# hasindu2008/squigulator

Measured on AMD Instinct MI355X. Metric: simulated raw samples/sec, higher is better.
Workload: dtype f32+f64

## Files before the change

squigulator_amd/csrc/h_common.h:

```cpp
#pragma once

#if defined(SQG_DEV)
#define SQG_DEV_ENV(name) getenv(name)
#else
#define SQG_DEV_ENV(name) (static_cast<const char*>(nullptr))
#endif
static inline int dev_env_int(const char* v, int dflt) { return v ? atoi(v) : dflt; }

#ifndef SQG_SOURCE_HASH
#define SQG_SOURCE_HASH "unstamped"
#endif
extern "C" const char sqg_source_hash_marker[] = "SQG_SOURCE_HASH=" SQG_SOURCE_HASH ";";
#if defined(SQG_DEV)
static const char kBuildInfo[] = "source_hash=" SQG_SOURCE_HASH ";dev=1";
#else
static const char kBuildInfo[] = "source_hash=" SQG_SOURCE_HASH ";dev=0";
#endif
extern "C" const char* sqg_build_info(void) { return kBuildInfo; }

#include "h_cpus.h"

static uint32_t lcg_pow(uint32_t base, unsigned long long e) {
    uint32_t r = 1, b = base;
    while (e) { if (e & 1) r = lcg_mul(r, b); b = lcg_mul(b, b); e >>= 1; }
// ... 69 lines not shown
        int* d_slow = nullptr; size_t slow_cap = 0;
        ItemDesc* d_items = nullptr; size_t items_cap = 0;
        uint32_t* d_part = nullptr; size_t part_cap = 0;
        uint32_t* d_lbase = nullptr; size_t lbase_cap = 0;
        int* d_tile_link = nullptr; size_t tile_link_cap = 0;
        uint32_t* d_part_state = nullptr; size_t part_state_cap = 0;
        hipEvent_t cal_a = nullptr, cal_b = nullptr; bool cal_pending = false; long long cal_events = 0; int cal_tries = 0; float cal_ps = 0.f;
        uint2* cal_prev = nullptr; float cal_prev_ps = 0.f;
        unsigned long long gen = 0;
        hipEvent_t done = nullptr;
        hipEvent_t sampled = nullptr;
    } slot[2];
    struct CountSet {
        uint16_t* d_dwell = nullptr; size_t dwell_cap = 0;
        uint32_t* d_tile_so = nullptr; size_t tile_cap = 0;
        unsigned long long* d_seglen = nullptr; size_t seglen_cap = 0;
        size_t seglen_dirty = 0;
        unsigned long long gen = 0;
    } cset[3];
    int num_cu = 256;
    std::deque<sqg_batch*> staged_q;
    hipStream_t fix_stream = nullptr;
    unsigned long long* d_scan_part = nullptr; size_t scan_part_cap = 0;
    uint32_t* d_link_rows = nullptr; size_t link_rows_cap = 0;
    uint32_t* d_pcnt[2] = {nullptr, nullptr}; size_t pcnt_cap[2] = {0, 0};
    uint32_t* d_slice = nullptr; size_t slice_cap = 0;
    uint32_t* d_phist = nullptr; size_t phist_cap = 0;
    double row_bound = 0;
    bool range_mode = false;
    uint32_t* d_xcounts = nullptr; size_t xcounts_cap = 0;
// ... 269 lines not shown
```

squigulator_amd/csrc/h_context.h:

```cpp
#pragma once

extern "C" const char* sqg_strerror(int code) {
    switch (code) {
    case SQG_OK: return "ok";
    case SQG_EINVAL: return "invalid argument or unsupported configuration";
    case SQG_ENOMEM: return "out of memory";
    case SQG_EDEVICE: return "HIP runtime error";
    case SQG_ESEQUENCE: return "batches must be run in staging order";
    case SQG_ENODEVICE: return "no usable HIP device";
    case SQG_EOVERFLOW: return "read too long (>= UINT32_MAX samples) or dwell > 65535";
    case SQG_EIO: return "file I/O error";
    default: return "unknown error";
    }
}

extern "C" const char* sqg_last_error(const sqg_ctx_t* ctx) { return ctx ? ctx->err.c_str() : ""; }

extern "C" int sqg_device_count(void) {
    int n = 0;
    if (hipGetDeviceCount(&n) != hipSuccess) return SQG_ENODEVICE;
    return n;
}

extern "C" int32_t sqg_worker_of(int32_t i, int32_t n_rec, int32_t T) {
    if (T <= 1 || n_rec <= 0) return 0;
    const int32_t step = (n_rec + T - 1) / T;
    return i / step;
}

extern "C" void sqg_destroy(sqg_ctx_t* ctx) {
    if (!ctx) return;
    if (ctx->b5_reader_drain) ctx->b5_reader_drain(ctx->b5_reader, true);
    (void)hipSetDevice(ctx->cfg.device);
    if (ctx->b5_stream) { (void)hipStreamSynchronize(ctx->b5_stream); (void)hipStreamDestroy(ctx->b5_stream); ctx->b5_stream = nullptr; }
    if (ctx->stream) (void)hipStreamSynchronize(ctx->stream);
    if (ctx->fix_stream) (void)hipStreamSynchronize(ctx->fix_stream);
    delete ctx->draw_ahead; ctx->draw_ahead = nullptr;
    (void)hipFree(ctx->d_pcnt[0]); (void)hipFree(ctx->d_pcnt[1]); (void)hipFree(ctx->d_slice); (void)hipFree(ctx->d_phist);
    (void)hipFree(ctx->d_rows); (void)hipFree(ctx->d_link_rows); (void)hipFree(ctx->d_scan_part); (void)hipFree(ctx->d_xcounts); (void)hipFree(ctx->d_model); (void)hipFree(ctx->d_samp_scratch); (void)hipFree(ctx->d_pow); (void)hipFree(ctx->d_err); (void)hipFree(ctx->d_mid_done); if (ctx->h_samp) (void)hipHostFree(ctx->h_samp);
    for (auto& Q : ctx->cset) { (void)hipFree(Q.d_dwell); (void)hipFree(Q.d_tile_so); (void)hipFree(Q.d_seglen); }
    for (auto& S : ctx->slot) {
        (void)hipFree(S.d_sig); (void)hipFree(S.d_sigoff);
        (void)hipFree(S.d_fix); (void)hipFree(S.d_fix_count); (void)hipFree(S.d_fix_sh); (void)hipFree(S.d_fix_sh_count);
        (void)hipFree(S.d_evrec); (void)hipFree(S.d_slow);
        (void)hipFree(S.d_items); (void)hipFree(S.d_part_state); (void)hipFree(S.d_part); (void)hipFree(S.d_lbase); (void)hipFree(S.d_tile_link);
        (void)hipFree(S.cal_prev);
        if (S.cal_a) (void)hipEventDestroy(S.cal_a);
        if (S.cal_b) (void)hipEventDestroy(S.cal_b);
        if (S.done) (void)hipEventDestroy(S.done);
        if (S.sampled) (void)hipEventDestroy(S.sampled);
    }
    (void)hipFree(ctx->d_svb); (void)hipFree(ctx->d_svb_size); (void)hipFree(ctx->d_svb_off);
    (void)hipFree(ctx->d_b5meta); (void)hipFree(ctx->d_b5out); (void)hipFree(ctx->d_b5tab); (void)hipFree(ctx->d_b5size); for (auto* q : ctx->h_b5out) if (q) (void)hipHostFree(q); if (ctx->h_b5meta) (void)hipHostFree(ctx->h_b5meta);
    (void)hipFree(ctx->d_chunk_off); (void)hipFree(ctx->d_chunk_const); (void)hipFree(ctx->d_chunk_read); (void)hipFree(ctx->d_chunk_ev); (void)hipFree(ctx->d_chunk_wide); (void)hipFree(ctx->d_chunk_ghist); (void)hipFree(ctx->d_target_start);
    (void)hipFree(ctx->d_genome); (void)hipFree(ctx->d_contig_off); (void)hipFree(ctx->d_cum); (void)hipFree(ctx->d_nprefix);
// ... 178 lines not shown
```

squigulator_amd/csrc/h_results.h:

```cpp
#pragma once

static bool slot_is_mine(const sqg_ctx* c, const sqg_batch* b) { return c->slot[b->slot].gen == b->slot_gen; }
static bool cset_is_mine(const sqg_ctx* c, const sqg_batch* b) { return c->cset[b->cset].gen == b->cset_gen; }

extern "C" int sqg_batch_wait(sqg_ctx_t* c, sqg_batch_t* b, sqg_result_t* res) {
    if (!c || !b || !b->ran) return SQG_EINVAL;
    HIPCHK(c, hipSetDevice(c->cfg.device));
    HIPCHK(c, hipEventSynchronize(b->ev[4]));
    sqg_ctx::Slot& S = c->slot[b->slot];
    if (!b->waited) {
        b->n_samples = b->h_sigoff[b->n];
        for (int i = 0; i <= b->n; i++) b->sig_off[(size_t)i] = b->h_sigoff[i];
        unsigned int e = 0;
        const unsigned int* const hres = reinterpret_cast<const unsigned int*>(b->h_sigoff + (b->h_n - SQG_HRES_LL));
        if (b->fixup_launched) e = hres[0];
        else HIPCHK(c, hipMemcpy(&e, b->d_err, sizeof e, hipMemcpyDeviceToHost));
        b->waited = true;
        if (e) {
            c->err = "device reported: " + std::string((e & 1) ? "dwell>65535 " : "") + ((e & 2) ? "read>=UINT32_MAX samples " : "") + ((e & 4) ? "internal length mismatch " : "") + ((e & 8) ? "FP64 fix-up list overflow " : "") + ((e & 32) ? "one k-mer stream asked for >= 2^32 samples by one batch " : "") +
                     ((e & 64) ? "LDS atomics were not served in lane order (the batch's sample of the stream hand-out; create the context with SQG_ORDER_FREE) " : "") +
                     ((e & 0x80000000u) ? "the batch's last kernel left no report" : "");
            b->wait_rc = (e & (12 | 64 | 0x80000000u)) ? SQG_EDEVICE : SQG_EOVERFLOW;
            return b->wait_rc;
        }
// ... 47 lines not shown

extern "C" int sqg_fetch_dwell(sqg_ctx_t* c, sqg_batch_t* b, int32_t* dst) {
    if (!c || !b || !b->ran || !dst) return SQG_EINVAL;
    if (b->run_idx + 2 < c->runs || !slot_is_mine(c, b) || !cset_is_mine(c, b)) return SQG_ESEQUENCE;
    HIPCHK(c, hipSetDevice(c->cfg.device));
    HIPCHK(c, hipEventSynchronize(b->ev[4]));
    if (!c->use_dwell_stream) {
        for (long long i = 0; i < b->n_events; i++) dst[i] = (int)c->cfg.profile.dwell_mean;
        return SQG_OK;
    }
    std::vector<uint16_t> tmp((size_t)b->n_events);
    if (b->n_events) HIPCHK(c, hipMemcpy(tmp.data(), c->cset[b->cset].d_dwell, tmp.size() * sizeof(uint16_t), hipMemcpyDeviceToHost));
    for (size_t i = 0; i < tmp.size(); i++) dst[i] = tmp[i];
    return SQG_OK;
}

extern "C" int sqg_get_timing(sqg_ctx_t* c, sqg_timing_t* t) {
    if (!c || !t) return SQG_EINVAL;
    *t = c->timing;
    return SQG_OK;
}

extern "C" int sqg_set_phase_timing(sqg_ctx_t* c, int every) {
    if (!c || every < 0) return SQG_EINVAL;
    c->phase_timing_every = every;
    return SQG_OK;
}

extern "C" int sqg_set_stage_threads(sqg_ctx_t* c, int n) {
    if (!c || n < 0 || n > 64) return SQG_EINVAL;
// ... 194 lines not shown
```

squigulator_amd/csrc/h_run.h:

```cpp
#pragma once

static void count_params(sqg_ctx* c, const sqg_batch* b, sqg_ctx::CountSet& Q, const int n_part, uint32_t* d_pcnt, SigParams& P) {
    const sqg_profile_t& p = c->cfg.profile;
    P.reads = b->d_reads; P.chain_off = b->d_chain_off; P.chain_reads = b->d_chain_reads; P.chain_order = b->d_chain_order; P.bases = b->d_bases;
    P.dwell = c->use_dwell_stream ? Q.d_dwell : nullptr; P.dwell_out = Q.d_dwell; P.seglen_out = Q.d_seglen; P.seglen = Q.d_seglen; P.tile_so = Q.d_tile_so;
    P.dmean = p.dwell_mean; P.dstd = p.dwell_std; P.pw = c->d_pow; P.err = b->d_err; P.delta_x = c->delta_x;
    P.k = c->k; P.num_kmer = c->num_kmer; P.const_sps = (int)p.dwell_mean;
    P.dwell_unbounded = c->dwell_hi > 65535.0 ? 1 : 0;
    P.dwell_pack = c->dwell_hi < 1024.0 ? 1 : 0;
    P.pieces = b->d_pieces; P.piece_total = b->d_piece_total;
    P.pcnt = d_pcnt; P.n_part = n_part; P.n_links = b->n_chains;
}

struct RunStep { const char* name; std::function<int()> go; };
typedef std::vector<RunStep> RunPlan;

struct Run {
    sqg_ctx* c; sqg_batch* b; int phase; const uint32_t* before; const uint32_t* after;
    sqg_ctx::Slot* S; sqg_ctx::Slot* other; sqg_ctx::CountSet* Q;
    int n = 0, n_part = 0, dw = 0;
    bool certified = false, direct = false, fold = false, untimed = false, wave_links = false;
    size_t n_pairs = 0, n_rows = 0;
    unsigned scan_wgs = 0, pgrid = 0;
    uint32_t *d_pcnt = nullptr, *slice_lo = nullptr, *slice_hi = nullptr, *pfirst = nullptr, *pstart = nullptr, *ptotal = nullptr;
// ... 103 lines not shown
    P.part = S.d_part; P.part_state = b->part ? S.d_part_state : nullptr;
    P.poff = b->one ? b->d_link_slot : R.d_pcnt ? R.d_pcnt + (size_t)b->n_chains * n_part : nullptr;
    P.link_q = b->d_link_q;
    P.one = b->one ? 1 : 0;
    count_params(c, b, Q, n_part, R.d_pcnt, P);
    P.pstart = R.pstart;
    P.sig_off = S.d_sigoff; P.model = c->d_model; P.rows = c->d_rows;
    P.seed_base = canon((long long)c->cfg.seed + (long long)c->wlo * ((long long)c->num_kmer + 10)); P.seed_step = canon((long long)c->num_kmer + 10);
    P.dig = p.digitisation; P.range = p.range; P.kd = p.digitisation / p.range;
    P.thr_all = c->thr_all;
    P.meth = (c->cfg.flags & SQG_METH) ? 1 : 0; P.num_kmer_pad = n_part * PART_SUB;
    P.meth_top = 1; for (int i = 1; i < c->k; i++) P.meth_top *= 5u;
    P.use_streams = c->use_kmer_streams ? 1 : 0;
    P.rna = (c->cfg.flags & SQG_RNA) ? 1 : 0;
    P.evrec = S.d_evrec;
    if (b->part && b->pieces && !b->one) { P.evrec32 = reinterpret_cast<uint32_t*>(S.d_evrec); P.lbase = S.d_lbase; P.tile_link = S.d_tile_link; }
    P.tile_read = b->d_tile_read; P.stile_read = b->d_stile_read;
    const bool rna_prefix = (c->cfg.flags & SQG_RNA) && (c->cfg.flags & SQG_PREFIX);
    P.shift_len = rna_prefix ? (int)strlen(kAdaptorRna) * (int)p.dwell_mean : 0;
    {
        const double v = 30 * p.digitisation / p.range;
        int32_t t = (v > -2147483649.0 && v < 2147483648.0) ? (int32_t)v : (int32_t)0x80000000u;
        P.shift = (int)(int16_t)(uint16_t)((uint32_t)t & 0xffffu);
    }
    P.slow_count = S.d_fix_count + 1; P.items = S.d_items; P.lean_epl = c->lean_epl;
    P.slow_tiles = (R.certified && c->use_kmer_streams) ? S.d_slow : nullptr;
    R.fold = phase == 0 && n > 0 && b->n_chains > 0 && b->part && !b->one && b->pieces && R.certified && c->use_kmer_streams;
    memset(&R.SA, 0, sizeof R.SA);
    if (n > 0 && phase != 1) {
        ScanArgs& SA = R.SA;
        SA.seglen = Q.d_seglen; SA.n_reads = n; SA.sig_off = S.d_sigoff; SA.host_off = b->h_sigoff_dev; SA.err = b->d_err; SA.counters = S.d_fix_count;
// ... 24 lines not shown
    const dim3 g((unsigned)((b->n_chains + PEV_WAVES - 1) / PEV_WAVES)), t(64 * PEV_WAVES);
    if (!count) hipLaunchKernelGGL((k_part_events<0, PEV_SCATTER>), dim3((unsigned)((b->n_chains + PEV_WAVES_SCATTER - 1) / PEV_WAVES_SCATTER)), dim3(64 * PEV_WAVES_SCATTER), 0, c->stream, P, b->n_chains, (uint32_t)b->n_events);
    else if (b->one) {
        if (dwm == 0) hipLaunchKernelGGL((k_part_events<0, PEV_ONE>), g, t, 0, c->stream, P, b->n_chains, (uint32_t)b->n_events);
        else if (dwm == 1) hipLaunchKernelGGL((k_part_events<1, PEV_ONE>), g, t, 0, c->stream, P, b->n_chains, (uint32_t)b->n_events);
        else hipLaunchKernelGGL((k_part_events<2, PEV_ONE>), g, t, 0, c->stream, P, b->n_chains, (uint32_t)b->n_events);
    }
    else if (dwm == 0) hipLaunchKernelGGL((k_part_events<0, PEV_COUNT>), g, t, 0, c->stream, P, b->n_chains, (uint32_t)b->n_events);
    else if (dwm == 1) hipLaunchKernelGGL((k_part_events<1, PEV_COUNT>), g, t, 0, c->stream, P, b->n_chains, (uint32_t)b->n_events);
    else hipLaunchKernelGGL((k_part_events<2, PEV_COUNT>), g, t, 0, c->stream, P, b->n_chains, (uint32_t)b->n_events);
}
#define PLACE_TRIES 3
static int place_calibrate(Run& R) {
    sqg_ctx* c = R.c; sqg_batch* b = R.b; sqg_ctx::Slot& S = *R.S;
    static const bool off = SQG_DEV_ENV("SQG_NO_PLACE") != nullptr;
    if (off || c->cal_runs_left <= 0 || !R.wave_links || !R.P.evrec32 || b->n_events < (1ll << 24)) return SQG_OK;
    if (!S.cal_a) { HIPCHK(c, hipEventCreate(&S.cal_a)); HIPCHK(c, hipEventCreate(&S.cal_b)); }
    if (S.cal_pending) {
        float ms = 0.f;
        HIPCHK(c, hipEventSynchronize(S.cal_b));
        HIPCHK(c, hipEventElapsedTime(&ms, S.cal_a, S.cal_b));
        S.cal_pending = false;
        float ps = ms * 1.0e9f / (float)S.cal_events;
        const char* what = "";
        if (S.cal_prev) {
            if (ps > S.cal_prev_ps) {
                HIPCHK(c, hipEventSynchronize(S.done));
                HIPCHK(c, hipFree(S.d_evrec));
                S.d_evrec = S.cal_prev; ps = S.cal_prev_ps; what = ": slower than the allocation before it, which is taken back";
                R.P.evrec = S.d_evrec; R.P.evrec32 = reinterpret_cast<uint32_t*>(S.d_evrec);
            } else { HIPCHK(c, hipFree(S.cal_prev)); what = ": kept"; }
            S.cal_prev = nullptr;
        }
        S.cal_ps = ps;
        if (getenv("SQG_VERBOSE")) fprintf(stderr, "[sqg] placement: slot %d scatter pass %.0f us = %.3f ps per event%s\n", b->slot, ms * 1.0e3f, ms * 1.0e9f / (float)S.cal_events, what);
        if (S.cal_tries < PLACE_TRIES && c->cal_runs_left >= 3 && S.d_evrec && S.evrec_cap) {
            uint2* fresh = nullptr;
            if (hipMalloc(&fresh, S.evrec_cap * sizeof(uint2)) == hipSuccess) {
                S.cal_prev = S.d_evrec; S.cal_prev_ps = S.cal_ps;
                S.d_evrec = fresh; S.cal_tries++;
                R.P.evrec = S.d_evrec; R.P.evrec32 = reinterpret_cast<uint32_t*>(S.d_evrec);
            } else (void)hipGetLastError();
        }
    }
    c->cal_runs_left--;
    return SQG_OK;
}

static void launch_rows_advance(Run& R) {
    sqg_ctx* c = R.c;
    const dim3 ag((unsigned)((R.n_rows + 255) / 256));
    if (R.direct) hipLaunchKernelGGL(k_rows_advance<true>, ag, dim3(256), 0, c->stream, c->d_rows, c->d_pow, R.n_rows, R.before, c->d_xcounts, R.after);
    else hipLaunchKernelGGL(k_rows_advance<false>, ag, dim3(256), 0, c->stream, c->d_rows, c->d_pow, R.n_rows, R.before, c->d_xcounts, R.after);
}

static void plan_first_pass(Run& R, RunPlan& plan) {
// ... 305 lines not shown
```

squigulator_amd/csrc/h_stage.h:

```cpp
#pragma once

extern "C" void sqg_batch_free(sqg_ctx_t* ctx, sqg_batch_t* b) {
    if (!b) return;
    if (ctx) {
        (void)hipSetDevice(ctx->cfg.device);
        if (b->ran && b->ev[4]) (void)hipEventSynchronize(b->ev[4]);
    }
    if (ctx && b->staged && !b->ran) {
        if ((b->begun || b->precounted) && ctx->stream) (void)hipStreamSynchronize(ctx->stream);
        ctx->abandoned.insert(b->seq);
    }
    if (ctx) for (auto it = ctx->staged_q.begin(); it != ctx->staged_q.end(); ++it) if (*it == b) { ctx->staged_q.erase(it); break; }
    if (ctx && !b->ran && ctx->stage_stream) (void)hipStreamSynchronize(ctx->stage_stream);
    if (b->h_svboff) (void)hipHostFree(b->h_svboff);
    if (ctx && b->d_block && b->h_sigoff && b->ev[0] && ctx->pool.size() < 4) {
        sqg_ctx::Recycled r;
        r.d_block = b->d_block; r.block_bytes = b->block_bytes; r.h_sigoff = b->h_sigoff; r.h_sigoff_dev = b->h_sigoff_dev; r.h_n = b->h_n;
        for (int i = 0; i < 8; i++) r.ev[i] = b->ev[i];
        r.h_meta = b->h_meta; r.h_meta_bytes = b->h_meta_bytes; r.ev_staged = b->ev_staged;
        ctx->pool.push_back(r);
    } else {
        (void)hipFree(b->d_block);
        if (b->h_sigoff) (void)hipHostFree(b->h_sigoff);
        if (b->h_meta) (void)hipHostFree(b->h_meta);
        for (auto& e : b->ev) if (e) (void)hipEventDestroy(e);
        if (b->ev_staged) (void)hipEventDestroy(b->ev_staged);
    }
    delete b;
}

static int grow_cset(sqg_ctx* c, sqg_ctx::CountSet& Q, const sqg_batch* b) {
    int rc2;
    const size_t n = (size_t)b->n;
    if (2 * (n + 1) > Q.seglen_cap) {
        if ((rc2 = ensure(c, (void**)&Q.d_seglen, &Q.seglen_cap, 2 * (n + 1 + n / 2), sizeof(unsigned long long)))) return rc2;
        Q.seglen_dirty = Q.seglen_cap / 2;
    }
    if ((rc2 = ensure(c, (void**)&Q.d_dwell, &Q.dwell_cap, (size_t)b->n_events + 1024, sizeof(uint16_t)))) return rc2;
    if ((rc2 = ensure(c, (void**)&Q.d_tile_so, &Q.tile_cap, (size_t)b->n_tiles + 64, sizeof(uint32_t)))) return rc2;
    return SQG_OK;
}
static int grow_slot(sqg_ctx* c, sqg_ctx::Slot& Z, const sqg_batch* b, bool with_output) {
    int rc2;
    const int n = b->n;
    const bool certified = c->cfg.mode == SQG_MODE_CERTIFIED;
    if ((size_t)n + 1 > Z.reads_cap) {
        HIPCHK(c, hipStreamSynchronize(c->stream));
        (void)hipFree(Z.d_sigoff); Z.d_sigoff = nullptr;
        const size_t cap = (size_t)n + 1 + (size_t)n / 2;
        HIPCHK(c, hipMalloc(&Z.d_sigoff, cap * sizeof(long long)));
        Z.reads_cap = cap;
    }
    if (Z.cal_prev && (size_t)b->n_events + 64 > Z.evrec_cap) {
        HIPCHK(c, hipStreamSynchronize(c->stream)); HIPCHK(c, hipStreamSynchronize(c->fix_stream));
// ... 520 lines not shown
```

squigulator_amd/csrc/k_common.h:

```cpp
#pragma once

#define LCG_M 2147483647u
#define LCG_A 16807u

#define POW_N 1024
#define POW_TABLES 5
#define POW_TOP 4096
#define POW_WORDS (4 * POW_N + POW_TOP)
#define LCG_ORD2 1073741823u

#define NEAR_ONE_BITS 17

__host__ __device__ static inline uint32_t lcg_mul(uint32_t a, uint32_t b) {
    const unsigned long long p = (unsigned long long)a * b;
    uint32_t r = (uint32_t)(p & LCG_M) + (uint32_t)(p >> 31);
    r = (r & LCG_M) + (r >> 31);
    return r;
}
__device__ static inline uint32_t lcg_mul_lazy(uint32_t a, uint32_t b) {
    const unsigned long long p = (unsigned long long)a * b;
    return (uint32_t)(p & LCG_M) + (uint32_t)(p >> 31);
}

__device__ static inline uint32_t lcg_mul_dbl(uint32_t a, uint32_t b2) {
// ... 89 lines not shown

struct ReadDesc {
    long long base_off;
    long long ev_off;
    double offset;
    int len0, len1;
    int ne0, ne1;
    int worker;
    uint32_t time_c0;
    int tile_off;
    int fast;
    int stile_off;
    int slot0;
};

struct FixEntry {
    long long at;
    long long ev;
    uint32_t c1;
    int read;
    int shifted;
    int pad;
};

struct ItemDesc {
    long long ev_first;
    long long sig_base;
    double offset;
    int n_ev;
    int n_samples;
    uint32_t at0;
    int ev_read0;
    int read;
    int shift_lo, shift_hi;
    int slot_first;
};

struct SigParams {
    const ReadDesc* reads;
    const int* chain_off;
    const int* chain_reads;
    const int* chain_order;
    const uint8_t* bases;
    const uint16_t* dwell;
    uint16_t* dwell_out;
    unsigned long long* seglen_out;
    int seglen_zero;
    double dmean, dstd;
    const unsigned long long* seglen;
    const long long* sig_off;
    const float2* model;
    const uint32_t* pw;
    uint32_t* rows;
    uint32_t* link_rows;
    uint32_t seed_base, seed_step;
    int16_t* sig;
    unsigned int* err;
    FixEntry* fix;
    unsigned int* fix_count;
    unsigned int fix_cap;
    FixEntry* fix_sh;
    unsigned int* fix_sh_count;
    unsigned int fix_sh_cap;
    unsigned int* fix_sh_stat;
    unsigned int* host_res;
    int fix_tag;
    uint2* evrec;
    uint32_t* evrec32;
    uint32_t* lbase;
    int* tile_link;
    uint32_t* tile_so;
    const int* tile_read;
    const int* stile_read;
    ItemDesc* items;
    int lean_epl;
    int* slow_tiles;
    unsigned int* slow_count;
    double dig, range, kd;
    float delta_x;
    float thr_all;
    int k, num_kmer;
    int meth;
    uint32_t meth_top;
// ... 30 lines not shown
```

squigulator_amd/csrc/k_part_events.h:

```cpp
#pragma once

#ifndef PEV_EPL
#define PEV_EPL 8
#endif
#define PEV_SEG (64 * PEV_EPL)
#define PEV_WAVES 4
#ifndef PEV_COUNT_OCC
#define PEV_COUNT_OCC 1
#endif
#define PEV_WAVES_SCATTER 2
#define PEV_HALO 24
#define PEV_WORDS ((PEV_SEG + PEV_HALO) / 16 + 2)

#define PEV_RING 32
#define PEV_LINE 16
#define PEV_TASKS (3 * PART_MAX)
#define PEV_FLUSH_IT 10
template <bool SCATTER>
struct PevWave {
    uint32_t codes[PEV_WORDS];
    uint32_t wslot[PART_MAX];
    uint32_t wbase[SCATTER ? PART_MAX : 1];
    uint32_t flu[SCATTER ? PART_MAX : 1];
    uint32_t ring[SCATTER ? PART_MAX * PEV_RING : 1];
    uint2 tasks[SCATTER ? PEV_TASKS : 1];
};
struct PevTables {
// ... 62 lines not shown
        for (int t0 = 4 * PEV_FLUSH_IT; t0 < n_task; t0 += 4) put(t0 + (lane >> 4));
        __builtin_amdgcn_wave_barrier();
        asm volatile("" ::: "memory");
    };
    const uint32_t a2seg = DW ? lcg_jump2(P.pw, (uint32_t)PEV_SEG) : 0u, a2half = DW ? lcg_jump2(P.pw, 256u) : 0u;
    const float dw_sf = (float)P.dstd, dw_mf = (float)P.dmean;
    const float dw_eps = P.delta_x * fabsf(dw_sf) + 4.0f * 5.9604645e-8f * (fabsf(dw_mf) + 7.0f * fabsf(dw_sf) + 1.0f) + 1e-6f;

    for (int ci = c_lo; ci < c_hi; ci++) {
        const int4 pc = P.pieces[ci];
        const int r = pc.x, e_lo = pc.y;
        const ReadDesc rd = P.reads[r];
        const int ne = pc.z;
        const bool whole = e_lo == 0 && ne == rd.ne0 + rd.ne1;
        const uint8_t* rbases = P.bases + rd.base_off;
        const int shift1 = rd.len0 - rd.ne0;
        unsigned long long done = 0;
        long long n1 = -1;
        uint32_t c_seg = DW ? (uint32_t)__builtin_amdgcn_readfirstlane((int)lcg_mul(lcg_mul(rd.time_c0, LCG_A), e_lo ? lcg_jump2(P.pw, (uint32_t)e_lo) : 1u)) : 0u;
        auto load8 = [&](const int bi) -> unsigned long long {
            unsigned long long v;
            __builtin_memcpy(&v, rbases + bi, 8);
            return v;
        };
        unsigned long long b_cur = 0, b_halo = 0;
        uint16_t d_cur[PEV_EPL];
        auto fetch = [&](const int s) {
            const int bs = s + (s >= rd.ne0 ? shift1 : 0);
            b_cur = load8(bs + 8 * lane);
            if (lane < PEV_HALO / 8) b_halo = load8(bs + PEV_SEG + 8 * lane);
            if (DW == 0 && P.dwell) {
#pragma unroll
                for (int q = 0; q < PEV_EPL; q++) d_cur[q] = P.dwell[rd.ev_off + s + 64 * q + lane];
            }
        };
#pragma unroll
        for (int q = 0; q < PEV_EPL; q++) d_cur[q] = 0;
        if (ne > e_lo) fetch(e_lo);
        __builtin_amdgcn_s_waitcnt(0x0F70);
        #define PEV_IN(j_) (FULL || (j_) < n_seg)
        auto segment = [&](auto full_tag, const int s0) {
            constexpr bool FULL = decltype(full_tag)::value;
            const int n_seg = FULL ? PEV_SEG : ne - s0;
            const bool second = s0 >= rd.ne0;
            {
                auto pack8 = [&](const unsigned long long v) -> uint32_t {
                    uint32_t h = 0;
#pragma unroll
                    for (int i = 0; i < 8; i++) h = (h << 2) | L.lut[(uint32_t)(v >> (8 * i)) & 0xffu];
                    return h;
                };
                reinterpret_cast<uint16_t*>(W.codes)[lane ^ 1] = (uint16_t)pack8(b_cur);
                if (lane < PEV_HALO / 8) reinterpret_cast<uint16_t*>(W.codes)[(64 + lane) ^ 1] = (uint16_t)pack8(b_halo);
            }
            int sps[PEV_EPL];
#pragma unroll
            for (int q = 0; q < PEV_EPL; q++) sps[q] = (DW == 0) ? (PEV_IN(64 * q + lane) ? (P.dwell ? (int)d_cur[q] : P.const_sps) : 0) : 0;
            if (s0 + PEV_SEG < ne) fetch(s0 + PEV_SEG);
            __builtin_amdgcn_wave_barrier();
            asm volatile("" ::: "memory");
            uint32_t rank[PEV_EPL];
            const bool straddle = SCATTER || (rd.ne1 > 0 && s0 < rd.ne0 && s0 + PEV_SEG > rd.ne0);
            if (!straddle) {
#pragma unroll
                for (int q = 0; q < PEV_EPL; q++) {
                    const int cb = 64 * q + lane;
                    const uint32_t hi = W.codes[cb >> 4], lo = W.codes[(cb >> 4) + 1];
                    rank[q] = (uint32_t)(((unsigned long long)hi << 32 | lo) >> (64 - 2 * (cb & 15) - 2 * k)) & kmask;
                }
            } else {
#pragma unroll
                for (int q = 0; q < PEV_EPL; q++) {
                    const int j = 64 * q + lane;
                    const int cb = j + ((!second && s0 + j >= rd.ne0) ? shift1 : 0);
                    const uint32_t hi = W.codes[cb >> 4], lo = W.codes[(cb >> 4) + 1];
                    rank[q] = (uint32_t)(((unsigned long long)hi << 32 | lo) >> (64 - 2 * (cb & 15) - 2 * k)) & kmask;
                }
            }
            uint32_t c_blk[PEV_EPL / 4];
            c_blk[0] = c_seg;
#pragma unroll
            for (int h = 1; h < PEV_EPL / 4; h++) c_blk[h] = DW ? (uint32_t)__builtin_amdgcn_readfirstlane((int)lcg_mul(c_blk[h - 1], a2half)) : 0u;
#pragma unroll
            for (int q = 0; q < PEV_EPL; q++) {
                const int j = 64 * q + lane;
                const bool valid = PEV_IN(j);
                if (DW != 0 && valid) {
                    const uint32_t c1 = lcg_mul_dbl(c_blk[q >> 2], L.jump[64 * (q & 3) + lane]);
                    bool decided = false;
                    int v = 0;
                    if (DW == 1) {
// ... 50 lines not shown
                done += run;
            } else {
                const uint32_t start = W.wslot[lane], flu = W.flu[lane];
                uint32_t slot[PEV_EPL];
                asm volatile("" ::: "memory");
#pragma unroll
                for (int q = 0; q < PEV_EPL; q++) {
                    slot[q] = 0;
                    if (PEV_IN(64 * q + lane)) slot[q] = __hip_atomic_fetch_add(&W.wslot[rank[q] >> PART_SUB_BITS], 1u, __ATOMIC_RELAXED, __HIP_MEMORY_SCOPE_WORKGROUP);
                    asm volatile("" ::: "memory");
                }
                const uint32_t end = W.wslot[lane];
#pragma unroll
                for (int q = 0; q < PEV_EPL; q++) {
                    if (PEV_IN(64 * q + lane))
                        __builtin_nontemporal_store((rank[q] << EVR_REL_BITS) | (slot[q] - W.wbase[rank[q] >> PART_SUB_BITS]), P.evrec32 + rd.ev_off + s0 + 64 * q + lane);
                }
                if (lane < PEV_EPL && s0 + 64 * lane < ne) P.tile_link[rd.tile_off + (s0 >> 6) + lane] = chain;
                if (__builtin_amdgcn_ballot_w64(end - flu > (uint32_t)PEV_RING) == 0ull) {
#pragma unroll
                    for (int q = 0; q < PEV_EPL; q++) {
                        if (PEV_IN(64 * q + lane))
                            W.ring[(rank[q] >> PART_SUB_BITS) * PEV_RING + (slot[q] & (PEV_RING - 1))] = (rank[q] & (PART_SUB - 1)) | ((uint32_t)sps[q] << 16);
                    }
                    const uint32_t upto = max(flu, end & ~(uint32_t)(PEV_LINE - 1));
                    W.flu[lane] = upto;
                    flush(flu, upto);
                } else {
                    flush(flu, start);
                    W.flu[lane] = end;
                    uint2* const sorted = reinterpret_cast<uint2*>(W.ring);
// ... 133 lines not shown
```

squigulator_amd/csrc/k_samples.h:

```cpp
#pragma once

struct SmpWaveLds {
    uint4 rec_a[64];
    uint2 rec_b[64];
    uint8_t mk[MK_W];
};
struct SmpLds {
    uint2 mult[MULT_N];
    SmpWaveLds w[4];
};

__device__ static inline void push_fix(const SigParams& P, bool bad, int lane, unsigned long long lane_le,
                                       long long at, uint32_t c1, long long ev, int r, int shifted) {
    const unsigned long long am = __ballot(bad);
    if (am) {
        unsigned int slot0 = 0;
        const int leader = __ffsll((long long)am) - 1;
        if (lane == leader) slot0 = atomicAdd(P.fix_count, (unsigned int)__popcll(am));
        slot0 = __shfl(slot0, leader);
        if (bad) {
            const unsigned int slot = slot0 + (unsigned int)__popcll(am & lane_le) - 1u;
            if (slot < P.fix_cap) {
                FixEntry fe; fe.at = at; fe.c1 = c1; fe.ev = ev; fe.read = r; fe.shifted = shifted; fe.pad = 0;
                P.fix[slot] = fe;
// ... 41 lines not shown
    if (!take) {
        const int nt = (n_ev + 63) >> 6;
        const unsigned int q = atomicAdd(P.slow_count, (unsigned int)nt);
        for (int i = 0; i < nt; i++) P.slow_tiles[q + i] = rd.tile_off + lt * LEAN_EPL + i;
    }
    ItemDesc d;
    d.ev_first = rd.ev_off + (long long)lt * LEAN_EV;
    d.sig_base = sig_base;
    d.offset = rd.offset;
    d.n_ev = (take && n_samples > 0) ? n_ev : 0;
    d.n_samples = n_samples;
    d.at0 = P.rna ? read_len - 1u - base_pos : base_pos;
    d.ev_read0 = lt * LEAN_EV;
    d.read = r;
    d.shift_lo = shift_lo; d.shift_hi = shift_hi;
    d.slot_first = P.one ? rd.slot0 + lt * LEAN_EV : P.evrec32 ? (rd.slot0 >= 0 ? rd.slot0 : P.tile_link[rd.tile_off + lt * LEAN_EPL]) : 0;
    P.items[g] = d;
}
__global__ __launch_bounds__(256) void k_items(const SigParams P, const int n_stiles) { items_body(P, (int)blockIdx.x, n_stiles); }

template <typename T>
__device__ static inline T sload(const T* p) {
    static_assert(sizeof(T) % 4 == 0, "dword granularity");
    const __attribute__((address_space(4))) uint32_t* src =
        reinterpret_cast<const __attribute__((address_space(4))) uint32_t*>(reinterpret_cast<uintptr_t>(p));
    uint32_t w[sizeof(T) / 4];
#pragma unroll
    for (int q = 0; q < (int)(sizeof(T) / 4); q++) w[q] = src[q];
    T v;
    __builtin_memcpy(&v, w, sizeof v);
    return v;
// ... 37 lines not shown
        int sps[LEAN_EPL];
        if (P.one) {
            const uint32_t gslot = (uint32_t)it.slot_first + (uint32_t)e0;
            if (e0 + LEAN_EPL <= ne) {
                uint32_t pw_[LEAN_EPL];
                __builtin_memcpy(pw_, P.part + gslot, 4 * LEAN_EPL);
#pragma unroll
                for (int q = 0; q < LEAN_EPL; q++) { er[q] = make_uint2(gslot + (uint32_t)q, pw_[q] & 0xffffu); sps[q] = (int)(pw_[q] >> 16); }
            } else {
#pragma unroll
                for (int q = 0; q < LEAN_EPL; q++) {
                    const uint32_t w_ = e0 + q < ne ? P.part[gslot + q] : 0u;
                    er[q] = make_uint2(gslot + (uint32_t)q, w_ & 0xffffu); sps[q] = (int)(w_ >> 16);
                }
            }
        } else if (P.evrec32) {
            const uint32_t lbv = P.lbase[(size_t)it.slot_first * PART_MAX + lane];
            uint32_t ew[LEAN_EPL];
            uint16_t dw[LEAN_EPL];
            __builtin_memcpy(ew, P.evrec32 + gev, 4 * LEAN_EPL);
            if (P.dwell) __builtin_memcpy(dw, P.dwell + gev, 2 * LEAN_EPL);
            else {
#pragma unroll
                for (int q = 0; q < LEAN_EPL; q++) dw[q] = (uint16_t)P.const_sps;
            }
#pragma unroll
            for (int q = 0; q < LEAN_EPL; q++) {
                const bool v = e0 + q < ne;
                const uint32_t rank = v ? ew[q] >> EVR_REL_BITS : 0u;
                const uint32_t lb_p = (uint32_t)__builtin_amdgcn_ds_bpermute((int)((rank >> PART_SUB_BITS) << 2), (int)lbv);
                er[q] = make_uint2(v ? lb_p + (ew[q] & ((1u << EVR_REL_BITS) - 1u)) : 0u, rank);
                sps[q] = v ? (int)dw[q] : 0;
            }
        } else if (e0 + LEAN_EPL <= ne) {
            uint32_t ew[2 * LEAN_EPL];
            __builtin_memcpy(ew, P.evrec + gev, 8 * LEAN_EPL);
#pragma unroll
            for (int q = 0; q < LEAN_EPL; q++) er[q] = make_uint2(ew[2 * q], ew[2 * q + 1]);
            if (P.dwell) {
                uint16_t dw[LEAN_EPL];
                __builtin_memcpy(dw, P.dwell + gev, 2 * LEAN_EPL);
#pragma unroll
                for (int q = 0; q < LEAN_EPL; q++) sps[q] = (int)dw[q];
            } else {
#pragma unroll
                for (int q = 0; q < LEAN_EPL; q++) sps[q] = P.const_sps;
// ... 149 lines not shown
    for (int wi = blockIdx.x * 4 + wid; wi < n_work; wi += gridDim.x * 4) {
        const int g = GENERIC && P.slow_tiles ? P.slow_tiles[wi] : wi;
        const int r = P.tile_read[g];
        const ReadDesc rd = P.reads[r];
        const int ne = rd.ne0 + rd.ne1;
        const int e = (g - rd.tile_off) * 64 + lane;
        const bool valid = e < ne;
        const long long ev_first = rd.ev_off + (long long)(g - rd.tile_off) * 64;
        uint2 er = make_uint2(0u, 0u);
        int sps = 0;
        if (valid) {
            if (P.one) {
                const uint32_t sl = (uint32_t)rd.slot0 + (uint32_t)e, w_ = P.part[sl];
                er = make_uint2(sl, w_ & 0xffffu);
                sps = (int)(w_ >> 16);
            } else if (P.evrec32) {
                const uint32_t w_ = P.evrec32[rd.ev_off + e], rank = w_ >> EVR_REL_BITS;
                er = make_uint2(P.lbase[(size_t)(rd.slot0 >= 0 ? rd.slot0 : P.tile_link[g]) * PART_MAX + (rank >> PART_SUB_BITS)] + (w_ & ((1u << EVR_REL_BITS) - 1u)), rank);
                sps = P.dwell ? (int)P.dwell[rd.ev_off + e] : P.const_sps;
            } else {
                er = P.evrec[rd.ev_off + e];
                sps = P.dwell ? (int)P.dwell[rd.ev_off + e] : P.const_sps;
            }
            if (P.part_state) er.x = P.part_state[er.x];
        }
        const float2 md = valid ? P.model[er.y] : make_float2(0.f, 0.f);
        const int incl = wave_incl_scan(sps, lane);
        const int wave_total = __shfl(incl, 63);
        const int so = incl - sps;
        const long long sig_base = P.sig_off[r];
        if (P.sig_off[r + 1] - sig_base >= 4294967295LL) continue;
        const uint32_t read_len = (uint32_t)(P.sig_off[r + 1] - sig_base);
        const long long n1 = (long long)P.seglen[2 * r];
// ... 183 lines not shown
```

Measured before the change: 576.2 billion.

## Store 16-bit event slot offsets and recompute k-mer ranks from packed base codes

The per-event record for the partitioned path shrinks from 32 bits (rank plus relative slot) to 16 bits (relative slot only). The k-mer rank is instead recomputed in the sample kernels from a new per-read packed 2-bit base code buffer, which the count pass writes out. This cuts event-record write and read traffic but adds a codes buffer, extra code writes in the count kernel, a larger halo, and rank recomputation with stall handling in the sample kernels. It also assumes relative slots fit in 16 bits.

```diff
diff --git a/squigulator_amd/csrc/h_common.h b/squigulator_amd/csrc/h_common.h
--- a/squigulator_amd/csrc/h_common.h
+++ b/squigulator_amd/csrc/h_common.h
@@ -107,6 +107,7 @@
     struct CountSet {
         uint16_t* d_dwell = nullptr; size_t dwell_cap = 0;
         uint32_t* d_tile_so = nullptr; size_t tile_cap = 0;
+        uint32_t* d_codes = nullptr; size_t codes_cap = 0;
         unsigned long long* d_seglen = nullptr; size_t seglen_cap = 0;
         size_t seglen_dirty = 0;
         unsigned long long gen = 0;
diff --git a/squigulator_amd/csrc/h_context.h b/squigulator_amd/csrc/h_context.h
--- a/squigulator_amd/csrc/h_context.h
+++ b/squigulator_amd/csrc/h_context.h
@@ -38,7 +38,7 @@
     delete ctx->draw_ahead; ctx->draw_ahead = nullptr;
     (void)hipFree(ctx->d_pcnt[0]); (void)hipFree(ctx->d_pcnt[1]); (void)hipFree(ctx->d_slice); (void)hipFree(ctx->d_phist);
     (void)hipFree(ctx->d_rows); (void)hipFree(ctx->d_link_rows); (void)hipFree(ctx->d_scan_part); (void)hipFree(ctx->d_xcounts); (void)hipFree(ctx->d_model); (void)hipFree(ctx->d_samp_scratch); (void)hipFree(ctx->d_pow); (void)hipFree(ctx->d_err); (void)hipFree(ctx->d_mid_done); if (ctx->h_samp) (void)hipHostFree(ctx->h_samp);
-    for (auto& Q : ctx->cset) { (void)hipFree(Q.d_dwell); (void)hipFree(Q.d_tile_so); (void)hipFree(Q.d_seglen); }
+    for (auto& Q : ctx->cset) { (void)hipFree(Q.d_dwell); (void)hipFree(Q.d_tile_so); (void)hipFree(Q.d_seglen); (void)hipFree(Q.d_codes); }
     for (auto& S : ctx->slot) {
         (void)hipFree(S.d_sig); (void)hipFree(S.d_sigoff);
         (void)hipFree(S.d_fix); (void)hipFree(S.d_fix_count); (void)hipFree(S.d_fix_sh); (void)hipFree(S.d_fix_sh_count);
diff --git a/squigulator_amd/csrc/h_results.h b/squigulator_amd/csrc/h_results.h
--- a/squigulator_amd/csrc/h_results.h
+++ b/squigulator_amd/csrc/h_results.h
@@ -85,6 +85,19 @@
     for (size_t i = 0; i < tmp.size(); i++) dst[i] = tmp[i];
     return SQG_OK;
 }
+
+#if defined(SQG_DEV)
+extern "C" int sqg_dev_fetch_codes(sqg_ctx_t* c, sqg_batch_t* b, uint32_t* dst, int64_t* first_word) {
+    if (!c || !b || !b->ran || !dst || !first_word) return SQG_EINVAL;
+    if (!(b->part && b->pieces && !b->one)) return SQG_EINVAL;
+    if (!cset_is_mine(c, b)) return SQG_ESEQUENCE;
+    HIPCHK(c, hipSetDevice(c->cfg.device));
+    HIPCHK(c, hipEventSynchronize(b->ev[4]));
+    for (int i = 0; i < b->n; i++) first_word[i] = (int64_t)(b->h_base_off[(size_t)i] >> 4) + i;
+    HIPCHK(c, hipMemcpy(dst, c->cset[b->cset].d_codes, (((size_t)b->n_bases >> 4) + (size_t)b->n) * sizeof(uint32_t), hipMemcpyDeviceToHost));
+    return SQG_OK;
+}
+#endif
 
 extern "C" int sqg_get_timing(sqg_ctx_t* c, sqg_timing_t* t) {
     if (!c || !t) return SQG_EINVAL;
diff --git a/squigulator_amd/csrc/h_run.h b/squigulator_amd/csrc/h_run.h
--- a/squigulator_amd/csrc/h_run.h
+++ b/squigulator_amd/csrc/h_run.h
@@ -3,6 +3,7 @@
 static void count_params(sqg_ctx* c, const sqg_batch* b, sqg_ctx::CountSet& Q, const int n_part, uint32_t* d_pcnt, SigParams& P) {
     const sqg_profile_t& p = c->cfg.profile;
     P.reads = b->d_reads; P.chain_off = b->d_chain_off; P.chain_reads = b->d_chain_reads; P.chain_order = b->d_chain_order; P.bases = b->d_bases;
+    P.codes = Q.d_codes;
     P.dwell = c->use_dwell_stream ? Q.d_dwell : nullptr; P.dwell_out = Q.d_dwell; P.seglen_out = Q.d_seglen; P.seglen = Q.d_seglen; P.tile_so = Q.d_tile_so;
     P.dmean = p.dwell_mean; P.dstd = p.dwell_std; P.pw = c->d_pow; P.err = b->d_err; P.delta_x = c->delta_x;
     P.k = c->k; P.num_kmer = c->num_kmer; P.const_sps = (int)p.dwell_mean;
@@ -141,7 +142,7 @@
     P.use_streams = c->use_kmer_streams ? 1 : 0;
     P.rna = (c->cfg.flags & SQG_RNA) ? 1 : 0;
     P.evrec = S.d_evrec;
-    if (b->part && b->pieces && !b->one) { P.evrec32 = reinterpret_cast<uint32_t*>(S.d_evrec); P.lbase = S.d_lbase; P.tile_link = S.d_tile_link; }
+    if (b->part && b->pieces && !b->one) { P.evrec16 = reinterpret_cast<uint16_t*>(S.d_evrec); P.lbase = S.d_lbase; P.tile_link = S.d_tile_link; }
     P.tile_read = b->d_tile_read; P.stile_read = b->d_stile_read;
     const bool rna_prefix = (c->cfg.flags & SQG_RNA) && (c->cfg.flags & SQG_PREFIX);
     P.shift_len = rna_prefix ? (int)strlen(kAdaptorRna) * (int)p.dwell_mean : 0;
@@ -196,7 +197,7 @@
 static int place_calibrate(Run& R) {
     sqg_ctx* c = R.c; sqg_batch* b = R.b; sqg_ctx::Slot& S = *R.S;
     static const bool off = SQG_DEV_ENV("SQG_NO_PLACE") != nullptr;
-    if (off || c->cal_runs_left <= 0 || !R.wave_links || !R.P.evrec32 || b->n_events < (1ll << 24)) return SQG_OK;
+    if (off || c->cal_runs_left <= 0 || !R.wave_links || !R.P.evrec16 || b->n_events < (1ll << 24)) return SQG_OK;
     if (!S.cal_a) { HIPCHK(c, hipEventCreate(&S.cal_a)); HIPCHK(c, hipEventCreate(&S.cal_b)); }
     if (S.cal_pending) {
         float ms = 0.f;
@@ -210,7 +211,7 @@
                 HIPCHK(c, hipEventSynchronize(S.done));
                 HIPCHK(c, hipFree(S.d_evrec));
                 S.d_evrec = S.cal_prev; ps = S.cal_prev_ps; what = ": slower than the allocation before it, which is taken back";
-                R.P.evrec = S.d_evrec; R.P.evrec32 = reinterpret_cast<uint32_t*>(S.d_evrec);
+                R.P.evrec = S.d_evrec; R.P.evrec16 = reinterpret_cast<uint16_t*>(S.d_evrec);
             } else { HIPCHK(c, hipFree(S.cal_prev)); what = ": kept"; }
             S.cal_prev = nullptr;
         }
@@ -221,7 +222,7 @@
             if (hipMalloc(&fresh, S.evrec_cap * sizeof(uint2)) == hipSuccess) {
                 S.cal_prev = S.d_evrec; S.cal_prev_ps = S.cal_ps;
                 S.d_evrec = fresh; S.cal_tries++;
-                R.P.evrec = S.d_evrec; R.P.evrec32 = reinterpret_cast<uint32_t*>(S.d_evrec);
+                R.P.evrec = S.d_evrec; R.P.evrec16 = reinterpret_cast<uint16_t*>(S.d_evrec);
             } else (void)hipGetLastError();
         }
     }
diff --git a/squigulator_amd/csrc/h_stage.h b/squigulator_amd/csrc/h_stage.h
--- a/squigulator_amd/csrc/h_stage.h
+++ b/squigulator_amd/csrc/h_stage.h
@@ -38,6 +38,8 @@
     }
     if ((rc2 = ensure(c, (void**)&Q.d_dwell, &Q.dwell_cap, (size_t)b->n_events + 1024, sizeof(uint16_t)))) return rc2;
     if ((rc2 = ensure(c, (void**)&Q.d_tile_so, &Q.tile_cap, (size_t)b->n_tiles + 64, sizeof(uint32_t)))) return rc2;
+    if (b->part && b->pieces && !b->one &&
+        (rc2 = ensure(c, (void**)&Q.d_codes, &Q.codes_cap, ((size_t)b->n_bases >> 4) + (size_t)b->n + CODE_SLACK, sizeof(uint32_t)))) return rc2;
     return SQG_OK;
 }
 static int grow_slot(sqg_ctx* c, sqg_ctx::Slot& Z, const sqg_batch* b, bool with_output) {
diff --git a/squigulator_amd/csrc/k_common.h b/squigulator_amd/csrc/k_common.h
--- a/squigulator_amd/csrc/k_common.h
+++ b/squigulator_amd/csrc/k_common.h
@@ -127,6 +127,12 @@
     int slot0;
 };
 
+__host__ __device__ static inline size_t code_origin(const ReadDesc& rd, const int r) { return (size_t)(rd.base_off >> 4) + (size_t)r; }
+#define CODE_SLACK 64
+__device__ static inline uint32_t code_rank(const uint32_t hi, const uint32_t lo, const int at, const int k, const uint32_t kmask) {
+    return (uint32_t)(((unsigned long long)hi << 32 | lo) >> (64 - 2 * at - 2 * k)) & kmask;
+}
+
 struct FixEntry {
     long long at;
     long long ev;
@@ -147,7 +153,10 @@
     int read;
     int shift_lo, shift_hi;
     int slot_first;
-};
+    uint32_t code_off;
+    int stall;
+};
+#define ITEM_NO_STALL (4095 << 4)
 
 struct SigParams {
     const ReadDesc* reads;
@@ -155,6 +164,7 @@
     const int* chain_reads;
     const int* chain_order;
     const uint8_t* bases;
+    uint32_t* codes;
     const uint16_t* dwell;
     uint16_t* dwell_out;
     unsigned long long* seglen_out;
@@ -179,7 +189,7 @@
     unsigned int* host_res;
     int fix_tag;
     uint2* evrec;
-    uint32_t* evrec32;
+    uint16_t* evrec16;
     uint32_t* lbase;
     int* tile_link;
     uint32_t* tile_so;
diff --git a/squigulator_amd/csrc/k_part_events.h b/squigulator_amd/csrc/k_part_events.h
--- a/squigulator_amd/csrc/k_part_events.h
+++ b/squigulator_amd/csrc/k_part_events.h
@@ -9,8 +9,9 @@
 #define PEV_COUNT_OCC 1
 #endif
 #define PEV_WAVES_SCATTER 2
-#define PEV_HALO 24
+#define PEV_HALO 40
 #define PEV_WORDS ((PEV_SEG + PEV_HALO) / 16 + 2)
+#define PEV_CODE_WORDS 34
 
 #define PEV_RING 32
 #define PEV_LINE 16
@@ -103,6 +104,7 @@
         const int ne = pc.z;
         const bool whole = e_lo == 0 && ne == rd.ne0 + rd.ne1;
         const uint8_t* rbases = P.bases + rd.base_off;
+        uint32_t* const rcodes = P.codes + code_origin(rd, r);
         const int shift1 = rd.len0 - rd.ne0;
         unsigned long long done = 0;
         long long n1 = -1;
@@ -113,11 +115,15 @@
             return v;
         };
         unsigned long long b_cur = 0, b_halo = 0;
+        uint32_t w_cur = 0;
         uint16_t d_cur[PEV_EPL];
         auto fetch = [&](const int s) {
-            const int bs = s + (s >= rd.ne0 ? shift1 : 0);
-            b_cur = load8(bs + 8 * lane);
-            if (lane < PEV_HALO / 8) b_halo = load8(bs + PEV_SEG + 8 * lane);
+            const int bs = (s + (s >= rd.ne0 ? shift1 : 0)) & ~15;
+            if (SCATTER) { if (lane < PEV_WORDS) w_cur = rcodes[(bs >> 4) + lane]; }
+            else {
+                b_cur = load8(bs + 8 * lane);
+                if (lane < PEV_HALO / 8) b_halo = load8(bs + PEV_SEG + 8 * lane);
+            }
             if (DW == 0 && P.dwell) {
 #pragma unroll
                 for (int q = 0; q < PEV_EPL; q++) d_cur[q] = P.dwell[rd.ev_off + s + 64 * q + lane];
@@ -132,7 +138,9 @@
             constexpr bool FULL = decltype(full_tag)::value;
             const int n_seg = FULL ? PEV_SEG : ne - s0;
             const bool second = s0 >= rd.ne0;
-            {
+            const int bs0 = s0 + (second ? shift1 : 0), b_at = bs0 & 15;
+            if (SCATTER) { if (lane < PEV_WORDS) W.codes[lane] = w_cur; }
+            else {
                 auto pack8 = [&](const unsigned long long v) -> uint32_t {
                     uint32_t h = 0;
 #pragma unroll
@@ -148,22 +156,27 @@
             if (s0 + PEV_SEG < ne) fetch(s0 + PEV_SEG);
             __builtin_amdgcn_wave_barrier();
             asm volatile("" ::: "memory");
+            if (MODE == PEV_COUNT) {
+                const int w0 = bs0 >> 4, n_read = rd.ne0 + rd.ne1;
+                const int i_lo = (s0 > 0 && b_at) ? 1 : 0;
+                const int nxt = s0 + PEV_SEG;
+                const int i_hi = min(nxt < n_read ? ((nxt + (nxt >= rd.ne0 ? shift1 : 0) + 15) >> 4) - w0 : ((rd.len0 + rd.len1 + 15) >> 4) - w0, PEV_CODE_WORDS);
+                if (lane >= i_lo && lane < i_hi) rcodes[w0 + lane] = W.codes[lane];
+            }
             uint32_t rank[PEV_EPL];
-            const bool straddle = SCATTER || (rd.ne1 > 0 && s0 < rd.ne0 && s0 + PEV_SEG > rd.ne0);
+            const bool straddle = SCATTER || b_at != 0 || (rd.ne1 > 0 && s0 < rd.ne0 && s0 + PEV_SEG > rd.ne0);
             if (!straddle) {
 #pragma unroll
                 for (int q = 0; q < PEV_EPL; q++) {
                     const int cb = 64 * q + lane;
-                    const uint32_t hi = W.codes[cb >> 4], lo = W.codes[(cb >> 4) + 1];
-                    rank[q] = (uint32_t)(((unsigned long long)hi << 32 | lo) >> (64 - 2 * (cb & 15) - 2 * k)) & kmask;
+                    rank[q] = code_rank(W.codes[cb >> 4], W.codes[(cb >> 4) + 1], cb & 15, k, kmask);
                 }
             } else {
 #pragma unroll
                 for (int q = 0; q < PEV_EPL; q++) {
                     const int j = 64 * q + lane;
-                    const int cb = j + ((!second && s0 + j >= rd.ne0) ? shift1 : 0);
-                    const uint32_t hi = W.codes[cb >> 4], lo = W.codes[(cb >> 4) + 1];
-                    rank[q] = (uint32_t)(((unsigned long long)hi << 32 | lo) >> (64 - 2 * (cb & 15) - 2 * k)) & kmask;
+                    const int cb = b_at + j + ((!second && s0 + j >= rd.ne0) ? shift1 : 0);
+                    rank[q] = code_rank(W.codes[cb >> 4], W.codes[(cb >> 4) + 1], cb & 15, k, kmask);
                 }
             }
             uint32_t c_blk[PEV_EPL / 4];
@@ -244,7 +257,7 @@
 #pragma unroll
                 for (int q = 0; q < PEV_EPL; q++) {
                     if (PEV_IN(64 * q + lane))
-                        __builtin_nontemporal_store((rank[q] << EVR_REL_BITS) | (slot[q] - W.wbase[rank[q] >> PART_SUB_BITS]), P.evrec32 + rd.ev_off + s0 + 64 * q + lane);
+                        __builtin_nontemporal_store((uint16_t)(slot[q] - W.wbase[rank[q] >> PART_SUB_BITS]), P.evrec16 + rd.ev_off + s0 + 64 * q + lane);
                 }
                 if (lane < PEV_EPL && s0 + 64 * lane < ne) P.tile_link[rd.tile_off + (s0 >> 6) + lane] = chain;
                 if (__builtin_amdgcn_ballot_w64(end - flu > (uint32_t)PEV_RING) == 0ull) {
diff --git a/squigulator_amd/csrc/k_samples.h b/squigulator_amd/csrc/k_samples.h
--- a/squigulator_amd/csrc/k_samples.h
+++ b/squigulator_amd/csrc/k_samples.h
@@ -79,7 +79,9 @@
     d.ev_read0 = lt * LEAN_EV;
     d.read = r;
     d.shift_lo = shift_lo; d.shift_hi = shift_hi;
-    d.slot_first = P.one ? rd.slot0 + lt * LEAN_EV : P.evrec32 ? (rd.slot0 >= 0 ? rd.slot0 : P.tile_link[rd.tile_off + lt * LEAN_EPL]) : 0;
+    d.slot_first = P.one ? rd.slot0 + lt * LEAN_EV : P.evrec16 ? (rd.slot0 >= 0 ? rd.slot0 : P.tile_link[rd.tile_off + lt * LEAN_EPL]) : 0;
+    d.code_off = (uint32_t)code_origin(rd, r);
+    d.stall = rd.ne1 > 0 ? (min(max(rd.ne0 - lt * LEAN_EV, 0), 4095) << 4) | (rd.len0 - rd.ne0) : ITEM_NO_STALL;
     P.items[g] = d;
 }
 __global__ __launch_bounds__(256) void k_items(const SigParams P, const int n_stiles) { items_body(P, (int)blockIdx.x, n_stiles); }
@@ -147,22 +149,38 @@
                     er[q] = make_uint2(gslot + (uint32_t)q, w_ & 0xffffu); sps[q] = (int)(w_ >> 16);
                 }
             }
-        } else if (P.evrec32) {
+        } else if (P.evrec16) {
             const uint32_t lbv = P.lbase[(size_t)it.slot_first * PART_MAX + lane];
-            uint32_t ew[LEAN_EPL];
-            uint16_t dw[LEAN_EPL];
-            __builtin_memcpy(ew, P.evrec32 + gev, 4 * LEAN_EPL);
+            uint16_t ew[LEAN_EPL], dw[LEAN_EPL];
+            uint32_t rk[LEAN_EPL];
+            __builtin_memcpy(ew, P.evrec16 + gev, 2 * LEAN_EPL);
             if (P.dwell) __builtin_memcpy(dw, P.dwell + gev, 2 * LEAN_EPL);
             else {
 #pragma unroll
                 for (int q = 0; q < LEAN_EPL; q++) dw[q] = (uint16_t)P.const_sps;
             }
+            const uint32_t* const cw = P.codes + it.code_off;
+            const uint32_t kmask = (1u << (2 * P.k)) - 1u;
+            const int st_at = it.stall >> 4, st_by = it.stall & 15;
+            if (st_at > 0 && st_at < ne) {
+#pragma unroll
+                for (int q = 0; q < LEAN_EPL; q++) {
+                    const int b = it.ev_read0 + e0 + q + (e0 + q >= st_at ? st_by : 0);
+                    rk[q] = code_rank(cw[b >> 4], cw[(b >> 4) + 1], b & 15, P.k, kmask);
+                }
+            } else {
+                const int b = it.ev_read0 + e0 + (st_at > 0 ? 0 : st_by);
+                uint32_t hl[2];
+                __builtin_memcpy(hl, cw + (b >> 4), 8);
+#pragma unroll
+                for (int q = 0; q < LEAN_EPL; q++) rk[q] = code_rank(hl[0], hl[1], (b & 15) + q, P.k, kmask);
+            }
 #pragma unroll
             for (int q = 0; q < LEAN_EPL; q++) {
                 const bool v = e0 + q < ne;
-                const uint32_t rank = v ? ew[q] >> EVR_REL_BITS : 0u;
+                const uint32_t rank = v ? rk[q] : 0u;
                 const uint32_t lb_p = (uint32_t)__builtin_amdgcn_ds_bpermute((int)((rank >> PART_SUB_BITS) << 2), (int)lbv);
-                er[q] = make_uint2(v ? lb_p + (ew[q] & ((1u << EVR_REL_BITS) - 1u)) : 0u, rank);
+                er[q] = make_uint2(v ? lb_p + (uint32_t)ew[q] : 0u, rank);
                 sps[q] = v ? (int)dw[q] : 0;
             }
         } else if (e0 + LEAN_EPL <= ne) {
@@ -342,9 +360,11 @@
                 const uint32_t sl = (uint32_t)rd.slot0 + (uint32_t)e, w_ = P.part[sl];
                 er = make_uint2(sl, w_ & 0xffffu);
                 sps = (int)(w_ >> 16);
-            } else if (P.evrec32) {
-                const uint32_t w_ = P.evrec32[rd.ev_off + e], rank = w_ >> EVR_REL_BITS;
-                er = make_uint2(P.lbase[(size_t)(rd.slot0 >= 0 ? rd.slot0 : P.tile_link[g]) * PART_MAX + (rank >> PART_SUB_BITS)] + (w_ & ((1u << EVR_REL_BITS) - 1u)), rank);
+            } else if (P.evrec16) {
+                const int cb = e + (e >= rd.ne0 ? rd.len0 - rd.ne0 : 0);
+                const uint32_t* const cw = P.codes + code_origin(rd, r) + (cb >> 4);
+                const uint32_t rank = code_rank(cw[0], cw[1], cb & 15, P.k, (1u << (2 * P.k)) - 1u);
+                er = make_uint2(P.lbase[(size_t)(rd.slot0 >= 0 ? rd.slot0 : P.tile_link[g]) * PART_MAX + (rank >> PART_SUB_BITS)] + (uint32_t)P.evrec16[rd.ev_off + e], rank);
                 sps = P.dwell ? (int)P.dwell[rd.ev_off + e] : P.const_sps;
             } else {
                 er = P.evrec[rd.ev_off + e];
```

After: 560.4 billion. 0.973x the previous value.
